# evgueni-ovtchinnikov/raleigh

Measured on AMD Instinct MI355X. Metric: inner-iter GB/s vs HBM roofline (Gram+dots+SpMM of one block-JCG iteration), higher is better.
Workload: dtype f64; 1 GPU; block-JCG inner iteration: 9 Gram + 4 dots + 1 SpMM, n=215x215x215=9938375 rows (9938375 per GPU), m=32, 7-pt Laplacian nnz=69291275, rows sharded over 1 GPU(s), strong scaling; n=9938375, m=32, nnz=69291275

## Files before the change

raleigh_amd/build.py:

```python

import hashlib
import os
import subprocess
import sys
from concurrent.futures import ThreadPoolExecutor

PKG = os.path.dirname(os.path.abspath(__file__))
ROOT = os.path.dirname(PKG)
CSRC = os.path.join(PKG, 'csrc')
LIBDIR = os.path.join(PKG, 'lib')
LIBPATH = os.path.join(LIBDIR, 'librlhip.so')
SOURCES = ['context', 'gram', 'update', 'spmm', 'spmm_wide_build', 'spmm_wide_s', 'spmm_wide_d', 'spmm_wide_c',
           'spmm_wide_z', 'sptrsv', 'dense', 'spmm_data']
HOST_SOURCES = ['ldlt_host', 'shm_reduce']
FLAGS = ['-O3', '--offload-arch=gfx950', '-fPIC', '-std=c++17', '-Wno-unused-result']


HASHPATH = LIBPATH + '.srchash'


def source_hash():
    files = sorted(os.path.join(CSRC, f) for f in os.listdir(CSRC))
    files.append(os.path.join(ROOT, 'include', 'rlhip.h'))
    h = hashlib.sha256(' '.join(FLAGS + SOURCES + HOST_SOURCES).encode())
    for f in files:
        h.update(os.path.basename(f).encode())
        with open(f, 'rb') as fh:
            h.update(fh.read())
    return h.hexdigest()


def is_up_to_date():
    if not (os.path.exists(LIBPATH) and os.path.exists(HASHPATH)):
        return False
    with open(HASHPATH) as fh:
        return fh.read().strip() == source_hash()


def build_library(force=False, verbose=False):
    if not force and is_up_to_date():
        return LIBPATH
    if os.path.exists(HASHPATH):
        os.remove(HASHPATH)
    hipcc = os.environ.get('HIPCC', 'hipcc')
    os.makedirs(LIBDIR, exist_ok=True)
    objdir = os.path.join(LIBDIR, 'obj')
    os.makedirs(objdir, exist_ok=True)
    inc = ['-I', os.path.join(ROOT, 'include'), '-I', CSRC]
# ... 28 lines not shown
```

raleigh_amd/csrc/common.h:

```cpp
#pragma once

#include <hip/hip_runtime.h>
#include <stdint.h>
#include <stdio.h>
#include <string.h>

#include <stdlib.h>

#include <string>
#include <thread>
#include <vector>

#include "rlhip.h"

namespace rlh {

void set_error(const char *fmt, ...);
int hip_fail(hipError_t e, const char *what, const char *file, int line);

#define RLH_HIP(call)                                                   \
  do {                                                                  \
    hipError_t e_ = (call);                                             \
    if (e_ != hipSuccess) return rlh::hip_fail(e_, #call, __FILE__, __LINE__); \
  } while (0)
// ... 43 lines not shown

__device__ __forceinline__ void fma_acc(float &acc, float a, float b)   { acc = fmaf(a, b, acc); }
__device__ __forceinline__ void fma_acc(double &acc, double a, double b) { acc = fma(a, b, acc); }
__device__ __forceinline__ void fma_acc(c32 &acc, c32 a, c32 b) {
  acc.re = fmaf(a.re, b.re, acc.re); acc.re = fmaf(-a.im, b.im, acc.re);
  acc.im = fmaf(a.re, b.im, acc.im); acc.im = fmaf(a.im, b.re, acc.im);
}
__device__ __forceinline__ void fma_acc(c64 &acc, c64 a, c64 b) {
  acc.re = fma(a.re, b.re, acc.re); acc.re = fma(-a.im, b.im, acc.re);
  acc.im = fma(a.re, b.im, acc.im); acc.im = fma(a.im, b.re, acc.im);
}
__device__ __forceinline__ void fma_conj_acc(float &acc, float a, float b)   { acc = fmaf(a, b, acc); }
__device__ __forceinline__ void fma_conj_acc(double &acc, double a, double b) { acc = fma(a, b, acc); }
__device__ __forceinline__ void fma_conj_acc(c32 &acc, c32 a, c32 b) {
  acc.re = fmaf(a.re, b.re, acc.re); acc.re = fmaf(a.im, b.im, acc.re);
  acc.im = fmaf(a.re, b.im, acc.im); acc.im = fmaf(-a.im, b.re, acc.im);
}
__device__ __forceinline__ void fma_conj_acc(c64 &acc, c64 a, c64 b) {
  acc.re = fma(a.re, b.re, acc.re); acc.re = fma(a.im, b.im, acc.re);
  acc.im = fma(a.re, b.im, acc.im); acc.im = fma(-a.im, b.re, acc.im);
}
__device__ __forceinline__ float  add_of(float a, float b)   { return a + b; }
__device__ __forceinline__ double add_of(double a, double b) { return a + b; }
__device__ __forceinline__ c32 add_of(c32 a, c32 b) { return c32{a.re + b.re, a.im + b.im}; }
__device__ __forceinline__ c64 add_of(c64 a, c64 b) { return c64{a.re + b.re, a.im + b.im}; }
__device__ __forceinline__ float  mul_of(float a, float b)   { return a * b; }
__device__ __forceinline__ double mul_of(double a, double b) { return a * b; }
__device__ __forceinline__ c32 mul_of(c32 a, c32 b) { return c32{a.re * b.re - a.im * b.im, a.re * b.im + a.im * b.re}; }
__device__ __forceinline__ c64 mul_of(c64 a, c64 b) { return c64{a.re * b.re - a.im * b.im, a.re * b.im + a.im * b.re}; }

constexpr int kRingSlots = 16;
constexpr size_t kRingSlotBytes = 1u << 20;
constexpr size_t kWorkspaceBytes = 96u << 20;

struct Context {
  bool ready = false;
  int device = -1;
  int num_cu = 256;
  hipStream_t own_stream = nullptr;
  hipStream_t stream = nullptr;
  char *ring_h = nullptr;
  char *ring_d = nullptr;
  hipEvent_t ring_ev[kRingSlots];
  bool ring_used[kRingSlots];
  int ring_next = 0;
  char *work = nullptr;
  char *result_d = nullptr;
  size_t result_d_bytes = 0;
  char *result_h = nullptr;
  char *result_hd = nullptr;
  size_t result_h_bytes = 0;
  hipEvent_t t0 = nullptr, t1 = nullptr;
  unsigned *async_err_h = nullptr;
  unsigned *async_err_d = nullptr;
};

Context &ctx();
int require_ready();
int check_async_error();

int ring_acquire(size_t bytes, int *slot, void **h, void **d);
int ring_commit(int slot, size_t bytes);
int ring_release(int slot);

int ensure_result(size_t bytes);
int fetch_result(void *h_out, const void *d_src, size_t bytes);

static inline bool aligned16(const void *p, int64_t ld, int64_t es) {
  return ((reinterpret_cast<uintptr_t>(p) & 15u) == 0) && (((ld * es) & 15) == 0);
}

}
```

raleigh_amd/csrc/context.hip:

```cpp
#include <stdarg.h>

#include "common.h"

namespace rlh {

static thread_local char g_err[1024] = "";

void set_error(const char *fmt, ...) {
  va_list ap;
  va_start(ap, fmt);
  vsnprintf(g_err, sizeof(g_err), fmt, ap);
  va_end(ap);
}

int hip_fail(hipError_t e, const char *what, const char *file, int line) {
  set_error("hip error %d (%s) in %s at %s:%d", (int)e, hipGetErrorString(e), what, file, line);
  return (int)e ? (int)e : 1;
}

int host_threads() {
  int t = env_int("RLH_HOST_THREADS", 0);
  if (t <= 0) {
    t = (int)std::thread::hardware_concurrency();
    if (t > 16) t = 16;
  }
  return t < 1 ? 1 : t;
}

Context &ctx() {
  static Context c;
  return c;
}

int require_ready() {
  if (!ctx().ready) {
    set_error("rlh_init() has not been called");
    return 1;
// ... 17 lines not shown
              bytes, kRingSlotBytes);
  int s = c.ring_next;
  c.ring_next = (s + 1) % kRingSlots;
  if (c.ring_used[s]) RLH_HIP(hipEventSynchronize(c.ring_ev[s]));
  *slot = s;
  *h = c.ring_h + (size_t)s * kRingSlotBytes;
  *d = c.ring_d + (size_t)s * kRingSlotBytes;
  return 0;
}

int ring_commit(int slot, size_t bytes) {
  Context &c = ctx();
  RLH_HIP(hipMemcpyAsync(c.ring_d + (size_t)slot * kRingSlotBytes, c.ring_h + (size_t)slot * kRingSlotBytes,
                         bytes, hipMemcpyHostToDevice, c.stream));
  return 0;
}

int ring_release(int slot) {
  Context &c = ctx();
  RLH_HIP(hipEventRecord(c.ring_ev[slot], c.stream));
  c.ring_used[slot] = true;
  return 0;
}

int ensure_result(size_t bytes) {
  Context &c = ctx();
  if (bytes > c.result_d_bytes) {
    size_t nb = bytes < (1u << 20) ? (1u << 20) : bytes * 2;
    RLH_HIP(hipStreamSynchronize(c.stream));
    if (c.result_d) RLH_HIP(hipFree(c.result_d));
    if (c.result_h) RLH_HIP(hipHostFree(c.result_h));
    c.result_d = nullptr; c.result_h = nullptr; c.result_hd = nullptr; c.result_d_bytes = c.result_h_bytes = 0;
    RLH_HIP(hipMalloc((void **)&c.result_d, nb));
    RLH_HIP(hipHostMalloc((void **)&c.result_h, nb, hipHostMallocMapped));
    RLH_HIP(hipHostGetDevicePointer((void **)&c.result_hd, c.result_h, 0));
    c.result_d_bytes = c.result_h_bytes = nb;
  }
  return 0;
}

int fetch_result(void *h_out, const void *d_src, size_t bytes) {
  Context &c = ctx();
  if (bytes == 0) return 0;
  if (d_src == c.result_hd && bytes <= c.result_h_bytes) {
    RLH_HIP(hipStreamSynchronize(c.stream));
    memcpy(h_out, c.result_h, bytes);
  } else if (bytes <= c.result_h_bytes) {
    RLH_HIP(hipMemcpyAsync(c.result_h, d_src, bytes, hipMemcpyDeviceToHost, c.stream));
    RLH_HIP(hipStreamSynchronize(c.stream));
    memcpy(h_out, c.result_h, bytes);
  } else {
    RLH_HIP(hipMemcpyAsync(h_out, d_src, bytes, hipMemcpyDeviceToHost, c.stream));
    RLH_HIP(hipStreamSynchronize(c.stream));
  }
  return check_async_error();
}

}

using namespace rlh;

extern "C" {

int rlh_version(void) { return RLH_VERSION; }

const char *rlh_last_error(void) { return g_err; }

int rlh_device_count(int *count) {
  RLH_REQUIRE(count != nullptr, "rlh_device_count: null argument");
  RLH_HIP(hipGetDeviceCount(count));
  return 0;
}

int rlh_init(int device) {
  Context &c = ctx();
  if (c.ready) {
    RLH_REQUIRE(c.device == device, "rlh_init: already bound to device %d (one device per process)", c.device);
    return 0;
  }
  int count = 0;
  RLH_HIP(hipGetDeviceCount(&count));
  RLH_REQUIRE(device >= 0 && device < count, "rlh_init: device %d out of range (%d visible)", device, count);
  RLH_HIP(hipSetDevice(device));
  hipDeviceProp_t prop;
  RLH_HIP(hipGetDeviceProperties(&prop, device));
  RLH_REQUIRE(strncmp(prop.gcnArchName, "gfx950", 6) == 0,
              "rlh_init: device %d is %s; this library is built for gfx950 (MI355X) only", device, prop.gcnArchName);
  c.num_cu = prop.multiProcessorCount;
  RLH_HIP(hipStreamCreateWithFlags(&c.own_stream, hipStreamNonBlocking));
  c.stream = c.own_stream;
  RLH_HIP(hipHostMalloc((void **)&c.ring_h, kRingSlots * kRingSlotBytes, hipHostMallocDefault));
  RLH_HIP(hipMalloc((void **)&c.ring_d, kRingSlots * kRingSlotBytes));
  for (int i = 0; i < kRingSlots; ++i) {
    RLH_HIP(hipEventCreateWithFlags(&c.ring_ev[i], hipEventDisableTiming));
    c.ring_used[i] = false;
  }
  RLH_HIP(hipMalloc((void **)&c.work, kWorkspaceBytes));
  RLH_HIP(hipEventCreate(&c.t0));
  RLH_HIP(hipEventCreate(&c.t1));
  RLH_HIP(hipHostMalloc((void **)&c.async_err_h, 64, hipHostMallocMapped));
  *c.async_err_h = 0;
  RLH_HIP(hipHostGetDevicePointer((void **)&c.async_err_d, c.async_err_h, 0));
  c.device = device;
  c.ready = true;
  if (int rc = ensure_result(1u << 20)) return rc;
  return 0;
}

int rlh_finalize(void) {
  Context &c = ctx();
  if (!c.ready) return 0;
  (void)hipStreamSynchronize(c.stream);
  for (int i = 0; i < kRingSlots; ++i) (void)hipEventDestroy(c.ring_ev[i]);
  (void)hipEventDestroy(c.t0);
  (void)hipEventDestroy(c.t1);
  (void)hipHostFree(c.ring_h);
  (void)hipFree(c.ring_d);
  (void)hipFree(c.work);
  if (c.result_d) (void)hipFree(c.result_d);
  if (c.result_h) (void)hipHostFree(c.result_h);
  if (c.async_err_h) (void)hipHostFree(c.async_err_h);
  (void)hipStreamDestroy(c.own_stream);
  c = Context();
  return 0;
}

int rlh_set_stream(void *hip_stream) {
  if (int rc = require_ready()) return rc;
  Context &c = ctx();
  RLH_HIP(hipStreamSynchronize(c.stream));
  c.stream = hip_stream ? (hipStream_t)hip_stream : c.own_stream;
  return 0;
}

int rlh_sync(void) {
  if (int rc = require_ready()) return rc;
  RLH_HIP(hipStreamSynchronize(ctx().stream));
  return check_async_error();
}

int rlh_mem_info(int64_t *free_bytes, int64_t *total_bytes) {
  if (int rc = require_ready()) return rc;
  size_t f = 0, t = 0;
  RLH_HIP(hipMemGetInfo(&f, &t));
  if (free_bytes) *free_bytes = (int64_t)f;
  if (total_bytes) *total_bytes = (int64_t)t;
  return 0;
}

int rlh_malloc(void **dptr, int64_t bytes) {
  if (int rc = require_ready()) return rc;
  RLH_REQUIRE(dptr != nullptr && bytes >= 0, "rlh_malloc: bad arguments");
  *dptr = nullptr;
  if (bytes == 0) return 0;
// ... 81 lines not shown
```

raleigh_amd/csrc/gram.hip:

```cpp
#include <stdlib.h>

#include "common.h"

namespace rlh {

template <typename R> struct Mfma16;
template <> struct Mfma16<double> {
  typedef double acc_t __attribute__((ext_vector_type(4)));
  static __device__ __forceinline__ acc_t run(double a, double b, acc_t c) {
    return __builtin_amdgcn_mfma_f64_16x16x4f64(a, b, c, 0, 0, 0);
  }
  static __device__ __forceinline__ int out_row(int lane, int reg) { return (lane >> 4) + 4 * reg; }
};
template <> struct Mfma16<float> {
  typedef float acc_t __attribute__((ext_vector_type(4)));
  static __device__ __forceinline__ acc_t run(float a, float b, acc_t c) {
    return __builtin_amdgcn_mfma_f32_16x16x4f32(a, b, c, 0, 0, 0);
  }
  static __device__ __forceinline__ int out_row(int lane, int reg) { return (lane >> 4) * 4 + reg; }
};

struct GramSeg { const void *p; int64_t ld; int c0; };
constexpr int kGramSegs = 4;

// ... 448 lines not shown
  Context &c = ctx();
  ZGramArgs a;
  a.X = (const c64 *)X; a.Y = (const c64 *)Y; a.ldx = ldx; a.ldy = ldy; a.n = n; a.mx = (int)mx; a.my = (int)my;
  a.nchunks = (n + kZgRows - 1) / kZgRows;
  a.partials = (double *)c.work;
  int64_t nb = c.num_cu;
  if (nb > a.nchunks) nb = a.nchunks;
  RLH_REQUIRE((size_t)nb * 64 * 128 * sizeof(double) <= kWorkspaceBytes, "rlh_gram: reduction workspace");
#define RLH_ZG(D_)                                                                                                  \
  do {                                                                                                              \
    static bool attr = false;                                                                                       \
    if (!attr) {                                                                                                    \
      RLH_HIP(hipFuncSetAttribute(reinterpret_cast<const void *>(&gram_z_dma_kernel<D_>),                           \
                                  hipFuncAttributeMaxDynamicSharedMemorySize, 2 * kZgBuf));                         \
      attr = true;                                                                                                  \
    }                                                                                                               \
    hipLaunchKernelGGL(gram_z_dma_kernel<D_>, dim3((unsigned)nb), dim3(1024), 2 * kZgBuf, c.stream, a);             \
  } while (0)
  switch (getenv("RLH_GRAM_ZDBG") ? atoi(getenv("RLH_GRAM_ZDBG")) : 0) {
    case 1: RLH_ZG(1); break;
    case 2: RLH_ZG(2); break;
    case 3: RLH_ZG(3); break;
    default: RLH_ZG(0); break;
  }
#undef RLH_ZG
  RLH_HIP(hipGetLastError());
  const int total = (int)(my * mx);
  hipLaunchKernelGGL(gram_z_finalize, dim3((total + 3) / 4), dim3(256), 0, c.stream, (const double *)c.work, (int)nb, (int)my,
                     (int)mx, (c64 *)d_out);
  RLH_HIP(hipGetLastError());
  return 0;
}

template <int DT>
__global__ __launch_bounds__(256) void gram_finalize(const void *partials_, int nbx, int npj, int VY, int VX, int my,
                                                     int mx, void *out_, int same) {
  using T = typename DType<DT>::T;
  using R = typename DType<DT>::R;
  constexpr bool CPLX = DType<DT>::cplx;
  constexpr int NCOMP = CPLX ? 4 : 1;
  const R *partials = reinterpret_cast<const R *>(partials_);
  const int lane = threadIdx.x & 63;
  const int e = blockIdx.x * 4 + (threadIdx.x >> 6);
  if (e >= my * mx) return;
  const int i = e / mx, j = e % mx;
  const int64_t slab = (int64_t)VY * VX;
  double t[NCOMP];
#pragma unroll
  for (int comp = 0; comp < NCOMP; ++comp) {
    int vi = CPLX ? 2 * i + (comp >> 1) : i;
    int vj = CPLX ? 2 * j + (comp & 1) : j;
    if (same && vi / VY == vj / VX && (vi % VY) / 16 > (vj % VX) / 16) { const int t_ = vi; vi = vj; vj = t_; }
    const int panel = (vi / VY) * npj + (vj / VX);
    const R *p = partials + ((int64_t)panel * slab + (vi % VY) * VX + (vj % VX)) * nbx;
    double s = 0.0;
    for (int b = lane; b < nbx; b += 64) s += (double)p[b];
#pragma unroll
    for (int off = 32; off > 0; off >>= 1) s += __shfl_xor(s, off);
    t[comp] = s;
  }
  if (lane == 0) {
    T *out = reinterpret_cast<T *>(out_);
    if constexpr (!CPLX) {
      out[e] = (R)t[0];
    } else {
      out[e].re = (R)(t[0] + t[3]);
      out[e].im = (R)(t[1] - t[2]);
    }
  }
}

template <int DT, int PI, int PJ, bool ALIGNED, int MODE, bool MULTI = false, bool QUAD = false, bool SYMS = false>
static int gram_blocks_per_cu() {
  static int cached = 0;
  if (cached == 0) {
    int nb = 0;
    if (hipOccupancyMaxActiveBlocksPerMultiprocessor(&nb, gram_kernel<DT, PI, PJ, ALIGNED, MODE, MULTI, QUAD, SYMS>, QUAD ? 512 : 256, 0) != hipSuccess ||
        nb < 1)
      nb = 1;
    cached = nb > 8 ? 8 : nb;
    const char *e = getenv("RLH_GRAM_WG_PER_CU");
    if (e && *e && atoi(e) > 0 && atoi(e) < cached) cached = atoi(e);
  }
  return cached;
}

static inline bool env_quad() {
  const char *e = getenv("RLH_GRAM_QUAD");
  return !(e && *e == '0');
}

static inline int pick_tiles(int v) {
  if (v <= 16) return 1;
  if (v <= 32) return 2;
  return 4;
}

template <int DT, int PI, int PJ, bool ALIGNED, int MODE, bool MULTI = false, bool QUAD = false, bool SYMS = false>
static int gram_launch(GramArgs &a, int npi, int npj, int64_t my, int64_t mx, void *d_out) {
  using R = typename DType<DT>::R;
  Context &c = ctx();
  constexpr int VY = PI * 16 * (QUAD ? 2 : 1), VX = PJ * 16 * (QUAD ? 4 : 1);
  const int npanels = npi * npj;
  int64_t nbx = (int64_t)c.num_cu * gram_blocks_per_cu<DT, PI, PJ, ALIGNED, MODE, MULTI, QUAD, SYMS>() / npanels;
  if (nbx < 1) nbx = 1;
  if (nbx > a.nchunks) nbx = a.nchunks;
  const size_t part_bytes = sizeof(R) * VY * VX;
  while (nbx > 1 && (size_t)nbx * npanels * part_bytes > kWorkspaceBytes) nbx /= 2;
  RLH_REQUIRE((size_t)nbx * npanels * part_bytes <= kWorkspaceBytes,
              "rlh_gram: %lld x %lld result exceeds the reduction workspace", (long long)my, (long long)mx);
  hipLaunchKernelGGL((gram_kernel<DT, PI, PJ, ALIGNED, MODE, MULTI, QUAD, SYMS>), dim3((unsigned)nbx, (unsigned)npanels), dim3(QUAD ? 512 : 256), 0,
                     c.stream, a);
  RLH_HIP(hipGetLastError());
  const int total = (int)(my * mx);
  hipLaunchKernelGGL((gram_finalize<DT>), dim3((total + 3) / 4), dim3(256), 0, c.stream, c.work, (int)nbx, npj, VY,
                     VX, (int)my, (int)mx, d_out, a.same);
  RLH_HIP(hipGetLastError());
  return 0;
}

static int gram_nt(int64_t bytes) {
  const char *e = getenv("RLH_GRAM_NT");
  if (e && *e) return atoi(e);
  return bytes > (int64_t)192 << 20;
}

constexpr int gram_stream_waves(int ncol) { return ncol <= 16 ? 16 : (ncol <= 32 ? 8 : 4); }

template <typename R, int TB, int NYC, int NXC, bool NT, bool XAL = false, bool CPLX = false>
__global__ __launch_bounds__(64 * (XAL ? 8 : gram_stream_waves(NYC + NXC))) void gram_stream_kernel(GramArgs a) {
  using M = Mfma16<R>;
  using acc_t = typename M::acc_t;
  constexpr bool SELF = NYC == 0;
  constexpr int RPU = 16 / (int)sizeof(R);
  constexpr int NP = TB / 16;
  constexpr int ROWS = NP * RPU;
  constexpr int NCOL = XAL ? NYC : NYC + NXC;
  constexpr int NC = CPLX ? 2 : 1;
  constexpr int NPT = NP * NC;
  constexpr int CPL = 64 / NPT;
  constexpr int NL = NCOL / NC / CPL;
  static_assert(!(CPLX && XAL) && NPT <= 64, "complex tiles");
  constexpr int KS = ROWS / 4;
  constexpr int SW = NP / 16;
  constexpr int PJ = NXC / 16, PI = SELF ? PJ : NYC / 16;
  static_assert(NP >= 16 && NP <= 64 && 64 % NP == 0 && NCOL % CPL == 0, "tile shape");
  constexpr int WPG = XAL ? 8 : gram_stream_waves(NYC + NXC);
  extern __shared__ __attribute__((aligned(16))) char lds_all[];
  char *lds = lds_all + (threadIdx.x >> 6) * (NCOL * TB);
// ... 209 lines not shown
    if (a.nt & 1) RLH_GS1(NYC_, NXC_, true); else RLH_GS1(NYC_, NXC_, false);                                          \
  } while (0)
  if (!CPLX && a.xal >= 0 && nyc == 64 && nxc == 32) {
    lds = (size_t)8 * 64 * TB;
    if (lds < (size_t)8 * 8 * 256 * sizeof(R)) lds = (size_t)8 * 8 * 256 * sizeof(R);
    if (lds < 84 * 1024) lds = 84 * 1024;
    nbx = c.num_cu;
    if (nbx * 8 > ntiles) nbx = (ntiles + 7) / 8;
    if (nbx < 1) nbx = 1;
    nparts_alias = nbx;
#define RLH_GSA(NT_)                                                                                                   \
  do {                                                                                                                 \
    static bool attr = false;                                                                                          \
    if (!attr) {                                                                                                       \
      RLH_HIP(hipFuncSetAttribute(reinterpret_cast<const void *>(&gram_stream_kernel<R, TB, 64, 32, NT_, true>),       \
                                  hipFuncAttributeMaxDynamicSharedMemorySize, 160 * 1024));                            \
      attr = true;                                                                                                     \
    }                                                                                                                  \
    hipLaunchKernelGGL((gram_stream_kernel<R, TB, 64, 32, NT_, true>), dim3((unsigned)nbx), dim3(64 * 8),                    \
                       lds, c.stream, a);                                                                              \
  } while (0)
    if (a.nt & 1) RLH_GSA(true); else RLH_GSA(false);
#undef RLH_GSA
  } else if (nxc == 16) {
    if (nyc == 0) RLH_GS(0, 16); else if (nyc == 16) RLH_GS(16, 16); else if (nyc == 32) RLH_GS(32, 16); else RLH_GS(64, 16);
  } else if (nxc == 32) {
    if (nyc == 0) RLH_GS(0, 32); else if (nyc == 16) RLH_GS(16, 32); else if (nyc == 32) RLH_GS(32, 32); else RLH_GS(64, 32);
  } else {
    if (nyc == 0) RLH_GS(0, 64); else RLH_GS(64, 64);
  }
#undef RLH_GS
#undef RLH_GS1
  RLH_HIP(hipGetLastError());
  const int total = (int)(my * mx);
  hipLaunchKernelGGL((gram_finalize<DT>), dim3((total + 3) / 4), dim3(256), 0, c.stream, c.work,
                     (int)(nparts_alias ? nparts_alias : nparts), 1, VY, nxc,
                     (int)my, (int)mx, d_out, a.same);
  RLH_HIP(hipGetLastError());
  return 0;
}

template <int DT>
static int gram_impl(int64_t n, int64_t mx, const void *X, int64_t ldx, int64_t my, const void *Y, int64_t ldy,
                     void *d_out) {
  using R = typename DType<DT>::R;
  constexpr int NC = DType<DT>::cplx ? 2 : 1;
  Context &c = ctx();
  const int vx = (int)mx * NC, vy = (int)my * NC;
  const int PI = pick_tiles(vy), PJ = pick_tiles(vx);
  const int npi = (vy + PI * 16 - 1) / (PI * 16), npj = (vx + PJ * 16 - 1) / (PJ * 16);
  GramArgs a;
  a.X = X; a.Y = Y; a.ldx = ldx; a.ldy = ldy; a.n = n; a.mx = (int)mx; a.my = (int)my;
  a.same = (X == Y && ldx == ldy && mx == my) ? 1 : 0;
  a.npj = npj; a.partials = c.work;
  const int64_t es = dtype_size(DT);
  a.nt = gram_nt(n * (a.same ? mx : mx + my) * es);
  const bool aligned = aligned16(X, ldx, es) && aligned16(Y, ldy, es);
  {
    const int stream = getenv("RLH_GRAM_STREAM") ? atoi(getenv("RLH_GRAM_STREAM")) : 1;
    if (stream && aligned && vx <= 64 && vy <= 64 && (vx > 8 || vy > 8)) {
      a.npj = 1;
      a.xal = -1;
      a.nxs = a.nys = 1;
      a.xs[0] = GramSeg{X, ldx, 0};
      a.ys[0] = GramSeg{Y, ldy, 0};
      for (int k = 1; k < kGramSegs; ++k) a.xs[k] = a.ys[k] = GramSeg{nullptr, 0, 1 << 30};
      return gram_stream_launch<DT>(a, my, mx, d_out);
    }
  }
  static const int pipe = getenv("RLH_GRAM_PIPE") ? atoi(getenv("RLH_GRAM_PIPE")) : 1;
// ... 133 lines not shown
      for (int i = 0; i < 4; ++i)
#pragma unroll
        for (int e = 0; e < VEC; ++e) fma_conj_acc(acc, xv[i].v[e], xv[i].v[e]);
    } else if (ALIGNED && base + 4 * 256 * VEC <= n) {
      V xv[4], yv[4];
#pragma unroll
      for (int i = 0; i < 4; ++i) {
        const int64_t r = base + ((int64_t)i * 256 + threadIdx.x) * VEC;
        xv[i] = piece(x + r);
        yv[i] = piece(y + r);
      }
#pragma unroll
      for (int i = 0; i < 4; ++i)
#pragma unroll
        for (int e = 0; e < VEC; ++e) fma_conj_acc(acc, yv[i].v[e], xv[i].v[e]);
    } else {
      for (int i = 0; i < 4; ++i) {
        const int64_t r = base + ((int64_t)i * 256 + threadIdx.x) * VEC;
        for (int e = 0; e < VEC && r + e < n; ++e) fma_conj_acc(acc, y[r + e], x[r + e]);
      }
    }
  }
  __shared__ T red[256];
  red[threadIdx.x] = acc;
  __syncthreads();
  for (int s = 128; s > 0; s >>= 1) {
    if (threadIdx.x < s) red[threadIdx.x] = add_of(red[threadIdx.x], red[threadIdx.x + s]);
    __syncthreads();
  }
  if (threadIdx.x == 0) partials[(int64_t)col * nbx + blockIdx.x] = red[0];
}

template <typename T>
__global__ __launch_bounds__(256) void dots_finalize(const T *partials, int nbx, int m, T *out) {
  const int lane = threadIdx.x & 63;
  const int col = blockIdx.x * 4 + (threadIdx.x >> 6);
  if (col >= m) return;
  T s = zero_of(T{});
  for (int b = lane; b < nbx; b += 64) s = add_of(s, partials[(int64_t)col * nbx + b]);
  if constexpr (sizeof(T) == sizeof(float) || sizeof(T) == sizeof(double)) {
    using R = T;
#pragma unroll
    for (int off = 32; off > 0; off >>= 1) s = s + (R)__shfl_xor(s, off);
  }
  if (lane == 0) out[col] = s;
}

template <typename R2, typename C>
__device__ __forceinline__ C shfl_complex(C v, int off) {
  C r;
  r.re = __shfl_xor(v.re, off);
  r.im = __shfl_xor(v.im, off);
  return r;
}

template <>
__global__ __launch_bounds__(256) void dots_finalize<c32>(const c32 *partials, int nbx, int m, c32 *out) {
  const int lane = threadIdx.x & 63;
  const int col = blockIdx.x * 4 + (threadIdx.x >> 6);
  if (col >= m) return;
  c32 s = zero_of(c32{});
  for (int b = lane; b < nbx; b += 64) s = add_of(s, partials[(int64_t)col * nbx + b]);
#pragma unroll
  for (int off = 32; off > 0; off >>= 1) s = add_of(s, shfl_complex<float>(s, off));
  if (lane == 0) out[col] = s;
}

template <>
__global__ __launch_bounds__(256) void dots_finalize<c64>(const c64 *partials, int nbx, int m, c64 *out) {
  const int lane = threadIdx.x & 63;
  const int col = blockIdx.x * 4 + (threadIdx.x >> 6);
  if (col >= m) return;
  c64 s = zero_of(c64{});
  for (int b = lane; b < nbx; b += 64) s = add_of(s, partials[(int64_t)col * nbx + b]);
#pragma unroll
  for (int off = 32; off > 0; off >>= 1) s = add_of(s, shfl_complex<double>(s, off));
  if (lane == 0) out[col] = s;
}

template <int DT>
static int dots_impl(int64_t n, int64_t m, const void *X, int64_t ldx, const void *Y, int64_t ldy, void *d_out) {
  using T = typename DType<DT>::T;
  Context &c = ctx();
  constexpr int VEC = 16 / (int)sizeof(T);
  int per = 4;
  int64_t nbx = (n + 256 * VEC * (int64_t)per - 1) / (256 * VEC * (int64_t)per);
  while (nbx > 2048 || (nbx > 1 && (size_t)nbx * m * sizeof(T) > kWorkspaceBytes / 4)) {
    per += 4;
    nbx = (n + 256 * VEC * (int64_t)per - 1) / (256 * VEC * (int64_t)per);
  }
  if (nbx < 1) nbx = 1;
  RLH_REQUIRE((size_t)nbx * m * sizeof(T) <= kWorkspaceBytes, "rlh_dots: too many columns");
  const int nt = gram_nt(n * m * (int64_t)sizeof(T) * (X == Y ? 1 : 2));
  const bool aligned = aligned16(X, ldx, sizeof(T)) && aligned16(Y, ldy, sizeof(T));
  dim3 grid((unsigned)nbx, (unsigned)m);
  if (aligned && (nt & 1))
    hipLaunchKernelGGL((dots_kernel<T, true, true>), grid, dim3(256), 0, c.stream, (const T *)X, ldx, (const T *)Y, ldy,
                       n, (T *)c.work, (int)nbx, per);
  else if (aligned)
    hipLaunchKernelGGL((dots_kernel<T, true, false>), grid, dim3(256), 0, c.stream, (const T *)X, ldx, (const T *)Y, ldy,
                       n, (T *)c.work, (int)nbx, per);
  else
    hipLaunchKernelGGL((dots_kernel<T, false, false>), grid, dim3(256), 0, c.stream, (const T *)X, ldx, (const T *)Y, ldy,
                       n, (T *)c.work, (int)nbx, per);
  RLH_HIP(hipGetLastError());
  hipLaunchKernelGGL((dots_finalize<T>), dim3(((int)m + 3) / 4), dim3(256), 0, c.stream, (const T *)c.work,
                     (int)nbx, (int)m, (T *)d_out);
  RLH_HIP(hipGetLastError());
  return 0;
}

template <typename R>
__global__ __launch_bounds__(256) void absmax_kernel(const R *X, int64_t ldx_r, int64_t n_r, double *partials, int nbx) {
  const R *x = X + (int64_t)blockIdx.y * ldx_r;
  double mx = 0.0;
  const int64_t stride = (int64_t)gridDim.x * 256;
  for (int64_t r = (int64_t)blockIdx.x * 256 + threadIdx.x; r < n_r; r += stride) {
    const double v = fabs((double)x[r]);
    mx = v > mx ? v : mx;
  }
  __shared__ double red[256];
  red[threadIdx.x] = mx;
  __syncthreads();
  for (int s = 128; s > 0; s >>= 1) {
    if (threadIdx.x < s) red[threadIdx.x] = red[threadIdx.x] > red[threadIdx.x + s] ? red[threadIdx.x] : red[threadIdx.x + s];
    __syncthreads();
  }
  if (threadIdx.x == 0) partials[(int64_t)blockIdx.y * nbx + blockIdx.x] = red[0];
}

__global__ __launch_bounds__(256) void absmax_finalize(const double *partials, int64_t count, double *out) {
  double mx = 0.0;
  for (int64_t i = threadIdx.x; i < count; i += 256) mx = partials[i] > mx ? partials[i] : mx;
  __shared__ double red[256];
  red[threadIdx.x] = mx;
  __syncthreads();
  for (int s = 128; s > 0; s >>= 1) {
    if (threadIdx.x < s) red[threadIdx.x] = red[threadIdx.x] > red[threadIdx.x + s] ? red[threadIdx.x] : red[threadIdx.x + s];
    __syncthreads();
  }
// ... 30 lines not shown
}

template <int DT>
static int dots_transp_impl(int64_t n, int64_t m, const void *X, int64_t ldx, const void *Y, int64_t ldy,
                            void *d_out) {
  using T = typename DType<DT>::T;
  Context &c = ctx();
  int64_t nb = (n + 255) / 256;
  if (nb > (int64_t)c.num_cu * 8) nb = (int64_t)c.num_cu * 8;
  hipLaunchKernelGGL((dots_transp_kernel<T>), dim3((unsigned)nb), dim3(256), 0, c.stream, (const T *)X, ldx,
                     (const T *)Y, ldy, n, (int)m, (T *)d_out);
  RLH_HIP(hipGetLastError());
  return 0;
}

}

using namespace rlh;

#define RLH_DISPATCH(dt, fn, ...)                              \
  switch (dt) {                                                \
    case RLH_S: rc = fn<RLH_S>(__VA_ARGS__); break;            \
    case RLH_D: rc = fn<RLH_D>(__VA_ARGS__); break;            \
    case RLH_C: rc = fn<RLH_C>(__VA_ARGS__); break;            \
    case RLH_Z: rc = fn<RLH_Z>(__VA_ARGS__); break;            \
    default: rlh::set_error("unknown dtype %d", dt); rc = 1;   \
  }

extern "C" {

int rlh_gram(int dtype, int64_t n, int64_t mx, const void *X, int64_t ldx, int64_t my, const void *Y, int64_t ldy,
             void *d_out, void *h_out) {
  if (int rc = require_ready()) return rc;
  RLH_REQUIRE(dtype_valid(dtype), "rlh_gram: unknown dtype %d", dtype);
  RLH_REQUIRE(n >= 0 && mx >= 0 && my >= 0, "rlh_gram: negative size");
  RLH_REQUIRE(mx <= 32768 && my <= 32768, "rlh_gram: more than 32768 vectors in a window");
  if (mx == 0 || my == 0) return 0;
  RLH_REQUIRE(X && Y, "rlh_gram: null block pointer");
  RLH_REQUIRE(ldx >= n && ldy >= n, "rlh_gram: leading dimension smaller than n");
  RLH_REQUIRE(d_out || h_out, "rlh_gram: no output buffer");
  const size_t bytes = (size_t)(mx * my * dtype_size(dtype));
  if (!d_out) {
    if (int rc = ensure_result(bytes)) return rc;
    d_out = ctx().result_hd;
  }
  int rc = 0;
  if (n == 0) {
    RLH_HIP(hipMemsetAsync(d_out, 0, bytes, ctx().stream));
  } else {
    RLH_DISPATCH(dtype, gram_impl, n, mx, X, ldx, my, Y, ldy, d_out)
  }
  if (rc) return rc;
  if (h_out) return fetch_result(h_out, d_out, bytes);
  return 0;
}

int rlh_gram_multi(int dtype, int64_t n, int nx, const void *const *X, const int64_t *ldx, const int64_t *mx, int ny,
                   const void *const *Y, const int64_t *ldy, const int64_t *my, void *d_out, void *h_out) {
  if (int rc = require_ready()) return rc;
  RLH_REQUIRE(dtype_valid(dtype), "rlh_gram_multi: unknown dtype %d", dtype);
  RLH_REQUIRE(nx >= 1 && nx <= kGramSegs && ny >= 1 && ny <= kGramSegs, "rlh_gram_multi: 1 to %d blocks per window", kGramSegs);
  RLH_REQUIRE(n >= 0 && X && ldx && mx && Y && ldy && my, "rlh_gram_multi: bad arguments");
  int64_t mxt = 0, myt = 0;
  for (int k = 0; k < nx; ++k) {
    RLH_REQUIRE(mx[k] >= 1 && X[k] && ldx[k] >= n, "rlh_gram_multi: bad block %d of the right window", k);
    mxt += mx[k];
  }
  for (int k = 0; k < ny; ++k) {
    RLH_REQUIRE(my[k] >= 1 && Y[k] && ldy[k] >= n, "rlh_gram_multi: bad block %d of the left window", k);
    myt += my[k];
  }
  RLH_REQUIRE(mxt <= 32768 && myt <= 32768, "rlh_gram_multi: more than 32768 vectors in a window");
  RLH_REQUIRE(d_out || h_out, "rlh_gram_multi: no output buffer");
  const size_t bytes = (size_t)(mxt * myt * dtype_size(dtype));
  if (!d_out) {
    if (int rc = ensure_result(bytes)) return rc;
    d_out = ctx().result_hd;
  }
  int rc = 0;
  if (n == 0) {
    RLH_HIP(hipMemsetAsync(d_out, 0, bytes, ctx().stream));
  } else {
    RLH_DISPATCH(dtype, gram_multi_impl, n, nx, X, ldx, mx, ny, Y, ldy, my, d_out)
  }
  if (rc) return rc;
  if (h_out) return fetch_result(h_out, d_out, bytes);
  return 0;
}

int rlh_dots(int dtype, int64_t n, int64_t m, const void *X, int64_t ldx, const void *Y, int64_t ldy, void *d_out,
             void *h_out) {
  if (int rc = require_ready()) return rc;
  RLH_REQUIRE(dtype_valid(dtype), "rlh_dots: unknown dtype %d", dtype);
  RLH_REQUIRE(n >= 0 && m >= 0, "rlh_dots: negative size");
  RLH_REQUIRE(m <= 32768, "rlh_dots: more than 32768 vectors in a window");
  if (m == 0) return 0;
  RLH_REQUIRE(X && Y, "rlh_dots: null block pointer");
  RLH_REQUIRE(ldx >= n && ldy >= n, "rlh_dots: leading dimension smaller than n");
  RLH_REQUIRE(d_out || h_out, "rlh_dots: no output buffer");
  const size_t bytes = (size_t)(m * dtype_size(dtype));
  if (!d_out) {
    if (int rc = ensure_result(bytes)) return rc;
    d_out = ctx().result_hd;
  }
  int rc = 0;
  if (n == 0) {
    RLH_HIP(hipMemsetAsync(d_out, 0, bytes, ctx().stream));
  } else {
    RLH_DISPATCH(dtype, dots_impl, n, m, X, ldx, Y, ldy, d_out)
  }
  if (rc) return rc;
  if (h_out) return fetch_result(h_out, d_out, bytes);
  return 0;
}

int rlh_absmax(int dtype, int64_t n, int64_t m, const void *X, int64_t ldx, double *h_out) {
  if (int rc = require_ready()) return rc;
  RLH_REQUIRE(dtype_valid(dtype), "rlh_absmax: unknown dtype %d", dtype);
  RLH_REQUIRE(n >= 0 && m >= 0 && m <= 65535, "rlh_absmax: bad size");
  RLH_REQUIRE(h_out != nullptr, "rlh_absmax: null output");
  if (n == 0 || m == 0) { *h_out = 0.0; return 0; }
  RLH_REQUIRE(X && ldx >= n, "rlh_absmax: bad block");
  if (int rc = ensure_result(sizeof(double))) return rc;
  void *d_out = ctx().result_hd;
  int rc = 0;
  RLH_DISPATCH(dtype, absmax_impl, n, m, X, ldx, d_out)
  if (rc) return rc;
  return fetch_result(h_out, d_out, sizeof(double));
}

int rlh_dots_transp(int dtype, int64_t n, int64_t m, const void *X, int64_t ldx, const void *Y, int64_t ldy,
                    void *d_out) {
  if (int rc = require_ready()) return rc;
  RLH_REQUIRE(dtype_valid(dtype), "rlh_dots_transp: unknown dtype %d", dtype);
  RLH_REQUIRE(n >= 0 && m >= 0, "rlh_dots_transp: negative size");
  if (n == 0) return 0;
  RLH_REQUIRE(d_out, "rlh_dots_transp: null output");
  RLH_REQUIRE(m == 0 || (X && Y), "rlh_dots_transp: null block pointer");
  RLH_REQUIRE(ldx >= n && ldy >= n, "rlh_dots_transp: leading dimension smaller than n");
  int rc = 0;
  RLH_DISPATCH(dtype, dots_transp_impl, n, m, X, ldx, Y, ldy, d_out)
  return rc;
}

}
```

Measured before the change: 6328 GB/s.

## Spin-wait on per-workgroup done flags instead of stream sync for host results

Finalize kernels now write results to coherent mapped host memory with system-scope atomic stores and publish a per-workgroup sequence flag. The host spins on these flags with a time budget and falls back to hipStreamSynchronize, so each Gram/dots result fetch avoids stream-sync latency. The dots finalize is also restructured to one block per column with a shared-memory tree reduction, and optional timing stamps and extra build flags are added. The cost is a busy-spinning host thread plus coherent host-memory traffic, with a risk of timeouts or ordering subtleties.

New measurement: 6315 GB/s. About the same (-0.2%).

```diff
diff --git a/raleigh_amd/build.py b/raleigh_amd/build.py
--- a/raleigh_amd/build.py
+++ b/raleigh_amd/build.py
@@ -14,6 +14,7 @@
            'spmm_wide_z', 'sptrsv', 'dense', 'spmm_data']
 HOST_SOURCES = ['ldlt_host', 'shm_reduce']
 FLAGS = ['-O3', '--offload-arch=gfx950', '-fPIC', '-std=c++17', '-Wno-unused-result']
+FLAGS += os.environ.get('RLH_BUILD_FLAGS', '').split()
 
 
 HASHPATH = LIBPATH + '.srchash'
diff --git a/raleigh_amd/csrc/common.h b/raleigh_amd/csrc/common.h
--- a/raleigh_amd/csrc/common.h
+++ b/raleigh_amd/csrc/common.h
@@ -99,6 +99,7 @@
 constexpr int kRingSlots = 16;
 constexpr size_t kRingSlotBytes = 1u << 20;
 constexpr size_t kWorkspaceBytes = 96u << 20;
+constexpr int kDoneWords = 1024;
 
 struct Context {
   bool ready = false;
@@ -117,6 +118,10 @@
   char *result_h = nullptr;
   char *result_hd = nullptr;
   size_t result_h_bytes = 0;
+  unsigned *done_h = nullptr;
+  unsigned *done_d = nullptr;
+  unsigned done_seq = 0;
+  int done_count = 0;
   hipEvent_t t0 = nullptr, t1 = nullptr;
   unsigned *async_err_h = nullptr;
   unsigned *async_err_d = nullptr;
@@ -131,7 +136,15 @@
 int ring_release(int slot);
 
 int ensure_result(size_t bytes);
+void result_publish(const void *d_out, int nwg, unsigned **words, unsigned *seq);
 int fetch_result(void *h_out, const void *d_src, size_t bytes);
+
+#ifdef RLH_STAMPS
+void stamp(int what);
+#else
+static inline void stamp(int) {}
+#endif
+enum { kStampEntry = 1, kStampMain = 2, kStampFinalize = 3, kStampAwake = 4, kStampReturn = 5 };
 
 static inline bool aligned16(const void *p, int64_t ld, int64_t es) {
   return ((reinterpret_cast<uintptr_t>(p) & 15u) == 0) && (((ld * es) & 15) == 0);
diff --git a/raleigh_amd/csrc/context.hip b/raleigh_amd/csrc/context.hip
--- a/raleigh_amd/csrc/context.hip
+++ b/raleigh_amd/csrc/context.hip
@@ -1,8 +1,32 @@
 #include <stdarg.h>
 
 #include "common.h"
+#include "result_wait.h"
 
 namespace rlh {
+
+#ifdef RLH_STAMPS
+namespace {
+struct Stamps {
+  struct E { int what; int64_t ns; };
+  std::vector<E> v;
+  Stamps() { v.reserve(1u << 20); }
+  ~Stamps() {
+    const char *f = getenv("RLH_STAMP_FILE");
+    FILE *fh = (f && *f) ? fopen(f, "w") : nullptr;
+    if (!fh) return;
+    for (const E &e : v) fprintf(fh, "%d %lld\n", e.what, (long long)e.ns);
+    fclose(fh);
+  }
+};
+Stamps g_stamps;
+}
+void stamp(int what) {
+  if (g_stamps.v.size() < g_stamps.v.capacity())
+    g_stamps.v.push_back({what, (int64_t)std::chrono::duration_cast<std::chrono::nanoseconds>(
+                                    std::chrono::steady_clock::now().time_since_epoch()).count()});
+}
+#endif
 
 static thread_local char g_err[1024] = "";
 
@@ -86,18 +110,47 @@
     if (c.result_h) RLH_HIP(hipHostFree(c.result_h));
     c.result_d = nullptr; c.result_h = nullptr; c.result_hd = nullptr; c.result_d_bytes = c.result_h_bytes = 0;
     RLH_HIP(hipMalloc((void **)&c.result_d, nb));
-    RLH_HIP(hipHostMalloc((void **)&c.result_h, nb, hipHostMallocMapped));
+    RLH_HIP(hipHostMalloc((void **)&c.result_h, nb, hipHostMallocMapped | hipHostMallocCoherent));
     RLH_HIP(hipHostGetDevicePointer((void **)&c.result_hd, c.result_h, 0));
     c.result_d_bytes = c.result_h_bytes = nb;
   }
   return 0;
 }
 
+static bool result_wait_spin() {
+  static const int spin = [] {
+    const char *e = getenv("RLH_RESULT_WAIT");
+    return (e && strcmp(e, "sync") == 0) ? 0 : 1;
+  }();
+  return spin != 0;
+}
+
+static int64_t result_spin_ns() {
+  static const int64_t ns = (int64_t)env_int("RLH_RESULT_SPIN_US", 4000) * 1000;
+  return ns;
+}
+
+void result_publish(const void *d_out, int nwg, unsigned **words, unsigned *seq) {
+  Context &c = ctx();
+  *words = nullptr;
+  *seq = 0;
+  c.done_count = 0;
+  if (d_out != c.result_hd || nwg < 1 || nwg > kDoneWords || !result_wait_spin()) return;
+  if (++c.done_seq == 0) c.done_seq = 1;
+  *words = c.done_d;
+  *seq = c.done_seq;
+  c.done_count = nwg;
+}
+
 int fetch_result(void *h_out, const void *d_src, size_t bytes) {
   Context &c = ctx();
   if (bytes == 0) return 0;
   if (d_src == c.result_hd && bytes <= c.result_h_bytes) {
-    RLH_HIP(hipStreamSynchronize(c.stream));
+    const int count = c.done_count;
+    c.done_count = 0;
+    if (count == 0 || !wait_words((const volatile uint32_t *)c.done_h, count, c.done_seq, result_spin_ns()))
+      RLH_HIP(hipStreamSynchronize(c.stream));
+    stamp(kStampAwake);
     memcpy(h_out, c.result_h, bytes);
   } else if (bytes <= c.result_h_bytes) {
     RLH_HIP(hipMemcpyAsync(c.result_h, d_src, bytes, hipMemcpyDeviceToHost, c.stream));
@@ -155,6 +208,9 @@
   RLH_HIP(hipHostMalloc((void **)&c.async_err_h, 64, hipHostMallocMapped));
   *c.async_err_h = 0;
   RLH_HIP(hipHostGetDevicePointer((void **)&c.async_err_d, c.async_err_h, 0));
+  RLH_HIP(hipHostMalloc((void **)&c.done_h, kDoneWords * sizeof(unsigned), hipHostMallocMapped | hipHostMallocCoherent));
+  memset(c.done_h, 0, kDoneWords * sizeof(unsigned));
+  RLH_HIP(hipHostGetDevicePointer((void **)&c.done_d, c.done_h, 0));
   c.device = device;
   c.ready = true;
   if (int rc = ensure_result(1u << 20)) return rc;
@@ -174,6 +230,7 @@
   if (c.result_d) (void)hipFree(c.result_d);
   if (c.result_h) (void)hipHostFree(c.result_h);
   if (c.async_err_h) (void)hipHostFree(c.async_err_h);
+  if (c.done_h) (void)hipHostFree(c.done_h);
   (void)hipStreamDestroy(c.own_stream);
   c = Context();
   return 0;
diff --git a/raleigh_amd/csrc/gram.hip b/raleigh_amd/csrc/gram.hip
--- a/raleigh_amd/csrc/gram.hip
+++ b/raleigh_amd/csrc/gram.hip
@@ -504,9 +504,33 @@
   return 0;
 }
 
+template <typename T>
+__device__ __forceinline__ void store_host(T *p, const T &v) {
+  if constexpr (sizeof(T) % 8 == 0) {
+    unsigned long long w[sizeof(T) / 8];
+    __builtin_memcpy(w, &v, sizeof(T));
+#pragma unroll
+    for (unsigned k = 0; k < sizeof(T) / 8; ++k)
+      __hip_atomic_store(reinterpret_cast<unsigned long long *>(p) + k, w[k], __ATOMIC_RELAXED, __HIP_MEMORY_SCOPE_SYSTEM);
+  } else {
+    unsigned w[sizeof(T) / 4];
+    __builtin_memcpy(w, &v, sizeof(T));
+#pragma unroll
+    for (unsigned k = 0; k < sizeof(T) / 4; ++k)
+      __hip_atomic_store(reinterpret_cast<unsigned *>(p) + k, w[k], __ATOMIC_RELAXED, __HIP_MEMORY_SCOPE_SYSTEM);
+  }
+  asm volatile("s_waitcnt vmcnt(0)" ::: "memory");
+}
+
+__device__ __forceinline__ void publish_done(unsigned *done, unsigned seq) {
+  if (!done) return;
+  __syncthreads();
+  if (threadIdx.x == 0) __hip_atomic_store(done + blockIdx.x, seq, __ATOMIC_RELAXED, __HIP_MEMORY_SCOPE_SYSTEM);
+}
+
 template <int DT>
 __global__ __launch_bounds__(256) void gram_finalize(const void *partials_, int nbx, int npj, int VY, int VX, int my,
-                                                     int mx, void *out_, int same) {
+                                                     int mx, void *out_, int same, unsigned *done, unsigned seq) {
   using T = typename DType<DT>::T;
   using R = typename DType<DT>::R;
   constexpr bool CPLX = DType<DT>::cplx;
@@ -514,7 +538,7 @@
   const R *partials = reinterpret_cast<const R *>(partials_);
   const int lane = threadIdx.x & 63;
   const int e = blockIdx.x * 4 + (threadIdx.x >> 6);
-  if (e >= my * mx) return;
+  if (e < my * mx) {
   const int i = e / mx, j = e % mx;
   const int64_t slab = (int64_t)VY * VX;
   double t[NCOMP];
@@ -533,13 +557,18 @@
   }
   if (lane == 0) {
     T *out = reinterpret_cast<T *>(out_);
+    T v;
     if constexpr (!CPLX) {
-      out[e] = (R)t[0];
+      v = (R)t[0];
     } else {
-      out[e].re = (R)(t[0] + t[3]);
-      out[e].im = (R)(t[1] - t[2]);
-    }
-  }
+      v.re = (R)(t[0] + t[3]);
+      v.im = (R)(t[1] - t[2]);
+    }
+    if (done) store_host(out + e, v);
+    else out[e] = v;
+  }
+  }
+  publish_done(done, seq);
 }
 
 template <int DT, int PI, int PJ, bool ALIGNED, int MODE, bool MULTI = false, bool QUAD = false, bool SYMS = false>
@@ -585,8 +614,10 @@
                      c.stream, a);
   RLH_HIP(hipGetLastError());
   const int total = (int)(my * mx);
+  unsigned *done, seq;
+  result_publish(d_out, (total + 3) / 4, &done, &seq);
   hipLaunchKernelGGL((gram_finalize<DT>), dim3((total + 3) / 4), dim3(256), 0, c.stream, c.work, (int)nbx, npj, VY,
-                     VX, (int)my, (int)mx, d_out, a.same);
+                     VX, (int)my, (int)mx, d_out, a.same, done, seq);
   RLH_HIP(hipGetLastError());
   return 0;
 }
@@ -862,10 +893,13 @@
 #undef RLH_GS
 #undef RLH_GS1
   RLH_HIP(hipGetLastError());
+  stamp(kStampMain);
   const int total = (int)(my * mx);
+  unsigned *done, seq;
+  result_publish(d_out, (total + 3) / 4, &done, &seq);
   hipLaunchKernelGGL((gram_finalize<DT>), dim3((total + 3) / 4), dim3(256), 0, c.stream, c.work,
                      (int)(nparts_alias ? nparts_alias : nparts), 1, VY, nxc,
-                     (int)my, (int)mx, d_out, a.same);
+                     (int)my, (int)mx, d_out, a.same, done, seq);
   RLH_HIP(hipGetLastError());
   return 0;
 }
@@ -1065,50 +1099,33 @@
 }
 
 template <typename T>
-__global__ __launch_bounds__(256) void dots_finalize(const T *partials, int nbx, int m, T *out) {
-  const int lane = threadIdx.x & 63;
-  const int col = blockIdx.x * 4 + (threadIdx.x >> 6);
-  if (col >= m) return;
+__global__ __launch_bounds__(256) void dots_finalize(const T *partials, int nbx, int m, T *out, unsigned *done,
+                                                     unsigned seq) {
+  const int col = blockIdx.x;
+  const T *p = partials + (int64_t)col * nbx;
   T s = zero_of(T{});
-  for (int b = lane; b < nbx; b += 64) s = add_of(s, partials[(int64_t)col * nbx + b]);
-  if constexpr (sizeof(T) == sizeof(float) || sizeof(T) == sizeof(double)) {
-    using R = T;
-#pragma unroll
-    for (int off = 32; off > 0; off >>= 1) s = s + (R)__shfl_xor(s, off);
-  }
-  if (lane == 0) out[col] = s;
-}
-
-template <typename R2, typename C>
-__device__ __forceinline__ C shfl_complex(C v, int off) {
-  C r;
-  r.re = __shfl_xor(v.re, off);
-  r.im = __shfl_xor(v.im, off);
-  return r;
-}
-
-template <>
-__global__ __launch_bounds__(256) void dots_finalize<c32>(const c32 *partials, int nbx, int m, c32 *out) {
-  const int lane = threadIdx.x & 63;
-  const int col = blockIdx.x * 4 + (threadIdx.x >> 6);
-  if (col >= m) return;
-  c32 s = zero_of(c32{});
-  for (int b = lane; b < nbx; b += 64) s = add_of(s, partials[(int64_t)col * nbx + b]);
-#pragma unroll
-  for (int off = 32; off > 0; off >>= 1) s = add_of(s, shfl_complex<float>(s, off));
-  if (lane == 0) out[col] = s;
-}
-
-template <>
-__global__ __launch_bounds__(256) void dots_finalize<c64>(const c64 *partials, int nbx, int m, c64 *out) {
-  const int lane = threadIdx.x & 63;
-  const int col = blockIdx.x * 4 + (threadIdx.x >> 6);
-  if (col >= m) return;
-  c64 s = zero_of(c64{});
-  for (int b = lane; b < nbx; b += 64) s = add_of(s, partials[(int64_t)col * nbx + b]);
-#pragma unroll
-  for (int off = 32; off > 0; off >>= 1) s = add_of(s, shfl_complex<double>(s, off));
-  if (lane == 0) out[col] = s;
+  for (int b0 = 0; b0 < nbx; b0 += 8 * 256) {
+    T v[8];
+#pragma unroll
+    for (int k = 0; k < 8; ++k) {
+      const int b = b0 + k * 256 + (int)threadIdx.x;
+      v[k] = b < nbx ? p[b] : zero_of(T{});
+    }
+#pragma unroll
+    for (int k = 0; k < 8; ++k) s = add_of(s, v[k]);
+  }
+  __shared__ T red[256];
+  red[threadIdx.x] = s;
+  __syncthreads();
+  for (int h = 128; h > 0; h >>= 1) {
+    if ((int)threadIdx.x < h) red[threadIdx.x] = add_of(red[threadIdx.x], red[threadIdx.x + h]);
+    __syncthreads();
+  }
+  if (threadIdx.x == 0) {
+    if (done) store_host(out + col, red[0]);
+    else out[col] = red[0];
+  }
+  publish_done(done, seq);
 }
 
 template <int DT>
@@ -1137,8 +1154,11 @@
     hipLaunchKernelGGL((dots_kernel<T, false, false>), grid, dim3(256), 0, c.stream, (const T *)X, ldx, (const T *)Y, ldy,
                        n, (T *)c.work, (int)nbx, per);
   RLH_HIP(hipGetLastError());
-  hipLaunchKernelGGL((dots_finalize<T>), dim3(((int)m + 3) / 4), dim3(256), 0, c.stream, (const T *)c.work,
-                     (int)nbx, (int)m, (T *)d_out);
+  stamp(kStampMain);
+  unsigned *done, seq;
+  result_publish(d_out, (int)m, &done, &seq);
+  hipLaunchKernelGGL((dots_finalize<T>), dim3((unsigned)m), dim3(256), 0, c.stream, (const T *)c.work,
+                     (int)nbx, (int)m, (T *)d_out, done, seq);
   RLH_HIP(hipGetLastError());
   return 0;
 }
@@ -1235,6 +1255,7 @@
 int rlh_gram(int dtype, int64_t n, int64_t mx, const void *X, int64_t ldx, int64_t my, const void *Y, int64_t ldy,
              void *d_out, void *h_out) {
   if (int rc = require_ready()) return rc;
+  stamp(kStampEntry);
   RLH_REQUIRE(dtype_valid(dtype), "rlh_gram: unknown dtype %d", dtype);
   RLH_REQUIRE(n >= 0 && mx >= 0 && my >= 0, "rlh_gram: negative size");
   RLH_REQUIRE(mx <= 32768 && my <= 32768, "rlh_gram: more than 32768 vectors in a window");
@@ -1245,6 +1266,7 @@
   const size_t bytes = (size_t)(mx * my * dtype_size(dtype));
   if (!d_out) {
     if (int rc = ensure_result(bytes)) return rc;
+    ctx().done_count = 0;
     d_out = ctx().result_hd;
   }
   int rc = 0;
@@ -1254,7 +1276,12 @@
     RLH_DISPATCH(dtype, gram_impl, n, mx, X, ldx, my, Y, ldy, d_out)
   }
   if (rc) return rc;
-  if (h_out) return fetch_result(h_out, d_out, bytes);
+  if (h_out) {
+    stamp(kStampFinalize);
+    rc = fetch_result(h_out, d_out, bytes);
+    stamp(kStampReturn);
+    return rc;
+  }
   return 0;
 }
 
@@ -1278,6 +1305,7 @@
   const size_t bytes = (size_t)(mxt * myt * dtype_size(dtype));
   if (!d_out) {
     if (int rc = ensure_result(bytes)) return rc;
+    ctx().done_count = 0;
     d_out = ctx().result_hd;
   }
   int rc = 0;
@@ -1294,6 +1322,7 @@
 int rlh_dots(int dtype, int64_t n, int64_t m, const void *X, int64_t ldx, const void *Y, int64_t ldy, void *d_out,
              void *h_out) {
   if (int rc = require_ready()) return rc;
+  stamp(kStampEntry);
   RLH_REQUIRE(dtype_valid(dtype), "rlh_dots: unknown dtype %d", dtype);
   RLH_REQUIRE(n >= 0 && m >= 0, "rlh_dots: negative size");
   RLH_REQUIRE(m <= 32768, "rlh_dots: more than 32768 vectors in a window");
@@ -1304,6 +1333,7 @@
   const size_t bytes = (size_t)(m * dtype_size(dtype));
   if (!d_out) {
     if (int rc = ensure_result(bytes)) return rc;
+    ctx().done_count = 0;
     d_out = ctx().result_hd;
   }
   int rc = 0;
@@ -1313,7 +1343,12 @@
     RLH_DISPATCH(dtype, dots_impl, n, m, X, ldx, Y, ldy, d_out)
   }
   if (rc) return rc;
-  if (h_out) return fetch_result(h_out, d_out, bytes);
+  if (h_out) {
+    stamp(kStampFinalize);
+    rc = fetch_result(h_out, d_out, bytes);
+    stamp(kStampReturn);
+    return rc;
+  }
   return 0;
 }
 
@@ -1325,6 +1360,7 @@
   if (n == 0 || m == 0) { *h_out = 0.0; return 0; }
   RLH_REQUIRE(X && ldx >= n, "rlh_absmax: bad block");
   if (int rc = ensure_result(sizeof(double))) return rc;
+  ctx().done_count = 0;
   void *d_out = ctx().result_hd;
   int rc = 0;
   RLH_DISPATCH(dtype, absmax_impl, n, m, X, ldx, d_out)
diff --git a/raleigh_amd/csrc/result_wait.h b/raleigh_amd/csrc/result_wait.h
--- /dev/null
+++ b/raleigh_amd/csrc/result_wait.h
@@ -0,0 +1,35 @@
+#pragma once
+
+#include <stdint.h>
+
+#include <chrono>
+
+#if defined(__x86_64__) || defined(__i386__)
+#include <immintrin.h>
+#endif
+
+namespace rlh {
+
+static inline void cpu_pause() {
+#if defined(__x86_64__) || defined(__i386__)
+  _mm_pause();
+#elif defined(__aarch64__)
+  __asm__ __volatile__("yield");
+#endif
+}
+
+static inline bool wait_words(const volatile uint32_t *words, int count, uint32_t seq, int64_t budget_ns) {
+  const auto t0 = std::chrono::steady_clock::now();
+  int seen = 0;
+  for (;;) {
+    for (int k = 0; k < 128; ++k) {
+      while (seen < count && __atomic_load_n(&words[seen], __ATOMIC_ACQUIRE) == seq) ++seen;
+      if (seen >= count) return true;
+      cpu_pause();
+    }
+    const int64_t ns = std::chrono::duration_cast<std::chrono::nanoseconds>(std::chrono::steady_clock::now() - t0).count();
+    if (ns >= budget_ns) return false;
+  }
+}
+
+}
```
